# ma921/SOBER

Hardware: AMD Instinct MI355X
Metric: recombination-step candidates/sec (N_rec=100000, N_nys=500, d=10, batch=100) (higher is better)
Workload: dtype f64

## Files before the change

sober_amd/csrc/car.hip:

```cpp
#include "common.hpp"
#include <atomic>
#include <cstdlib>

namespace sober {

constexpr int CAR_MS = 7;
constexpr int CAR_CQ = 13;
constexpr int CAR_NS = 16 * CAR_CQ;
constexpr int CAR_PC = 128;
constexpr int CAR_BT = 256;

template <int CTRL>
__device__ __forceinline__ double dpp(double v) {
    int lo = __double2loint(v), hi = __double2hiint(v);
    lo = __builtin_amdgcn_mov_dpp(lo, CTRL, 0xf, 0xf, true);
    hi = __builtin_amdgcn_mov_dpp(hi, CTRL, 0xf, 0xf, true);
    return __hiloint2double(hi, lo);
}
constexpr int ROR1 = 0x121, ROR2 = 0x122, ROR4 = 0x124, ROR8 = 0x128;

#define CAR_LDS_BARRIER() do { __builtin_amdgcn_s_waitcnt(0xC07F); __builtin_amdgcn_s_barrier(); } while (0)

__device__ __forceinline__ double row16_sum(double v) {
    v += dpp<ROR8>(v);
    v += dpp<ROR4>(v);
    v += dpp<ROR2>(v);
    v += dpp<ROR1>(v);
    return v;
}
__device__ __forceinline__ double grp8_sum(double v) {
    v += dpp<ROR8>(v);
    v += dpp<ROR4>(v);
    v += dpp<ROR2>(v);
    return v;
}
__device__ __forceinline__ double rdlane(double v, int l) {
    const int lo = __builtin_amdgcn_readlane(__double2loint(v), l);
    const int hi = __builtin_amdgcn_readlane(__double2hiint(v), l);
    return __hiloint2double(hi, lo);
}
__device__ __forceinline__ double wave_sum(double v) {
    v = row16_sum(v);
    return ((rdlane(v, 0) + rdlane(v, 16)) + rdlane(v, 32)) + rdlane(v, 48);
}

template <int CTRL, int ROW_MASK>
__device__ __forceinline__ unsigned long long dpp_u64(unsigned long long v) {
    int lo = (int)(unsigned)v, hi = (int)(unsigned)(v >> 32);
    lo = __builtin_amdgcn_update_dpp(lo, lo, CTRL, ROW_MASK, 0xf, false);
    hi = __builtin_amdgcn_update_dpp(hi, hi, CTRL, ROW_MASK, 0xf, false);
    return ((unsigned long long)(unsigned)hi << 32) | (unsigned)lo;
}
constexpr int BCAST15 = 0x142, BCAST31 = 0x143;

__device__ __forceinline__ unsigned long long ratio_key(double x) {
    const unsigned long long b = (unsigned long long)__double_as_longlong(x);
    const unsigned long long k = (b >> 63) ? ~b : (b | 0x8000000000000000ull);
    return (x != x) ? 0ull : k;
}

__device__ __forceinline__ double car_rcp(double c) {
    double r = __builtin_amdgcn_rcp(c);
    double e = fma(-c, r, 1.0);
    r = fma(r, e, r);
    e = fma(-c, r, 1.0);
    return fma(r, e, r);
}
__device__ __forceinline__ void amin_take(double& best, int& piv, double ob, int op) {
    const bool bn = best != best, on = ob != ob;
    const bool lt = (ob < best) | ((ob == best) & (op < piv));
    const bool nn = on & ((!bn) | (op < piv));
    const bool take = (op >= 0) & ((piv < 0) | ((bn | on) ? nn : lt));
    best = take ? ob : best;
    piv = take ? op : piv;
}


typedef unsigned int car_u32x4 __attribute__((ext_vector_type(4)));
typedef unsigned int car_u32x2 __attribute__((ext_vector_type(2)));
typedef __amdgpu_buffer_rsrc_t car_rsrc_t;
constexpr unsigned CARF_ERR = 0, CARF_XCD = 16, CARF_TICKET = 32, CARF_PROGRESS = 48, CARF_DONE = 56;
__host__ __device__ constexpr int64_t carf_bytes(int) { return 64; }
constexpr unsigned CARF_SPIN_LIMIT = 1u << 22;
__device__ __forceinline__ void carf_put(car_rsrc_t rs, unsigned off, double v, unsigned tag) {
    car_u32x4 g;
    g.x = (unsigned)__double2loint(v); g.y = tag; g.z = (unsigned)__double2hiint(v); g.w = tag;
    __builtin_amdgcn_raw_buffer_store_b128(g, rs, off, 0, 0);
}
__device__ __forceinline__ car_u32x4 carf_load(car_rsrc_t rs, unsigned off) {
    return __builtin_amdgcn_raw_buffer_load_b128(rs, off, 0, 16);
}
__device__ __forceinline__ bool carf_ok(const car_u32x4& g, unsigned tag) { return (g.y == tag) & (g.w == tag); }
__device__ __forceinline__ double carf_val(const car_u32x4& g) { return __hiloint2double((int)g.z, (int)g.x); }
struct CarPub { car_rsrc_t rs; unsigned tag0; };
__device__ __forceinline__ void car_publish_progress(const CarPub& pub, int k) {
    const int tid = threadIdx.x;
    if (k > 0 && (tid >> 6) == (((k - 1) & 15) >> 2)) {
        __builtin_amdgcn_s_waitcnt(0x0F70);
        if ((tid & 63) == 0) __builtin_amdgcn_raw_buffer_store_b32(pub.tag0 + (unsigned)k, pub.rs, CARF_PROGRESS, 0, 0);
    }
}

#ifdef CAR_BSTAMPS
#define CB_DECL unsigned long long cacc_[10] = {0, 0, 0, 0, 0, 0, 0, 0, 0, 0}, ctl_; \
    asm volatile("s_memtime %0\n\ts_waitcnt lgkmcnt(0)" : "=s"(ctl_) :: "memory");
#define CB_STAMP(K) do { unsigned long long t_; asm volatile("s_memtime %0\n\ts_waitcnt lgkmcnt(0)" : "=s"(t_) :: "memory"); \
    cacc_[K] += t_ - ctl_; ctl_ = t_; } while (0)
#define CB_FLUSH(S_) do { if ((threadIdx.x & 63) == 0) for (int k_ = 0; k_ < 10; ++k_) \
    ((unsigned long long*)(taup + 128 + CAR_NS * CAR_PC))[((threadIdx.x >> 6) * 8 + (S_)) * 10 + k_] = cacc_[k_]; } while (0)
#else
#define CB_DECL
#define CB_STAMP(K) do { } while (0)
#define CB_FLUSH(S_) do { } while (0)
#endif

struct CarLds2 {
    double* rowg; double* colg; double* zpart; double* s2part; double* zsum; double* scal; double* hsc;
};

#define CB2_RSUM(v) row16_sum(v)
#define CB2_HUPD(n, o) (n)
#define CB2_GUPD(n, o) (n)
#define CB2_BARRIER() CAR_LDS_BARRIER()
#define CB2_VSTORE(e) e
#ifdef CAR_BSTAMPS
#define CB2_STAMP(K, VAL) do { unsigned long long t_; asm volatile("s_memtime %0\n\ts_waitcnt lgkmcnt(0)" : "=s"(t_), "+v"(VAL) :: "memory"); \
    cacc_[K] += t_ - ctl_; ctl_ = t_; } while (0)
#else
#define CB2_STAMP(K, VAL) do { } while (0)
#endif
template <int S, bool FUSED, int MS, int CQ>
__device__ __forceinline__ void car_bidiag2_block(double (&a)[CAR_MS][CAR_CQ], double (&colp)[CAR_MS], int m, const CarLds2& L,
                                                  double* __restrict__ vws, double* __restrict__ taup, const CarPub& pub) {
    const int tid = threadIdx.x;
    const int R = tid >> 4, C = tid & 15;
    const int i_end = min(16 * S + 16, m - 1);
    constexpr int S1 = (S + 1 < MS) ? S + 1 : S;
    const car_rsrc_t vrs = __builtin_amdgcn_make_buffer_rsrc(vws, 0, (int)((size_t)m * CAR_NS * sizeof(double)), 0x00020000);
    CB_DECL
    for (int i = 16 * S; i < i_end; ++i) {
        const int li = i & 15, p = i & 1, pp = p ^ 1;
        if constexpr (FUSED) car_publish_progress(pub, i);
        double z[CAR_CQ], x[CAR_CQ], f[CAR_MS], cur[CAR_MS];
        CB_STAMP(0);
        const double tauq = L.hsc[0], sc2 = L.hsc[1];
#pragma unroll
        for (int q = S; q < CQ; ++q) { x[q] = L.rowg[pp * CAR_NS + C + 16 * q]; z[q] = L.zsum[C + 16 * q]; }
        const double rgi = L.rowg[pp * CAR_NS + i];
#pragma unroll
        for (int k = S; k < MS; ++k) cur[k] = L.colg[pp * 128 + R + 16 * k];
#pragma unroll
        for (int q = S; q < CQ; ++q) {
            z[q] = fma(sc2, z[q], x[q]);
            x[q] = fma(-tauq, z[q], x[q]);
        }
        z[S] = (C >= li) ? z[S] : 0.0;
        x[S] = (C > li) ? x[S] : 0.0;
#pragma unroll
        for (int k = S; k < MS; ++k) f[k] = tauq * (sc2 * colp[k]);
        f[S] = (R == li) ? tauq : f[S];
        const double zi = rdlane(z[S], li);
        const double alpha = fma(-tauq, zi, rgi);
#pragma unroll
        for (int k = S; k < MS; ++k) cur[k] = fma(-f[k], zi, cur[k]);
#pragma unroll
        for (int q = S; q < CQ; ++q)
#pragma unroll
            for (int k = S; k < MS; ++k) a[k][q] = CB2_HUPD(fma(-f[k], z[q], a[k][q]), a[k][q]);
        double ss0 = 0.0, ss1 = 0.0;
#pragma unroll
        for (int q = S; q < CQ; ++q) { if (q & 1) ss1 = fma(x[q], x[q], ss1); else ss0 = fma(x[q], x[q], ss0); }
        double ss = CB2_RSUM(ss0 + ss1);
        CB2_STAMP(2, ss);
        double beta, tau, sc;
        larfg_vt(alpha, ss, tau, sc); (void)beta;
        CB2_STAMP(3, tau);
        double tG[CAR_MS];
#pragma unroll
        for (int k = S; k < MS; ++k) {
            double w0 = 0.0, w1 = 0.0;
#pragma unroll
            for (int q = S; q < CQ; ++q) { if (q & 1) w1 = fma(a[k][q], x[q], w1); else w0 = fma(a[k][q], x[q], w0); }
            tG[k] = tau * fma(sc, CB2_RSUM(w0 + w1), cur[k]);
        }
        tG[S] = (R > li) ? tG[S] : 0.0;
        CB2_STAMP(4, tG[S]);
#pragma unroll
        for (int k = S; k < MS; ++k) colp[k] = cur[k] - tG[k];
        colp[S] = (R > li) ? colp[S] : 0.0;
#pragma unroll
        for (int q = S; q < CQ; ++q) x[q] *= sc;
        if (R == li) {
            const unsigned so = (unsigned)__builtin_amdgcn_readfirstlane(i) * (unsigned)(CAR_NS * 8);
            unsigned c8 = (unsigned)C * 8u;
            asm volatile("" : "+v"(c8));
#pragma unroll
            for (int q = 0; q < CAR_CQ; ++q) {
                double v;
                if (q < S || q >= CQ) v = 0.0;
                else if (q == S) v = (C < li) ? 0.0 : ((C == li) ? 1.0 : x[S]);
                else v = x[q];
                car_u32x2 g;
                g.x = (unsigned)__double2loint(v); g.y = (unsigned)__double2hiint(v);
                CB2_VSTORE(__builtin_amdgcn_raw_buffer_store_b64(g, vrs, c8 + (unsigned)(128 * q), so, 0));
            }
            if (C == 0) taup[i] = tau;
        }
#pragma unroll
        for (int k = S; k < MS; ++k)
#pragma unroll
            for (int q = S; q < CQ; ++q) a[k][q] = CB2_GUPD(fma(-tG[k], x[q], a[k][q]), a[k][q]);
        const bool last = li == 15;
        const int n1 = (li + 1) & 15;
        if (!last) {
            if (R == n1) {
#pragma unroll
                for (int q = S; q < CQ; ++q) L.rowg[p * CAR_NS + C + 16 * q] = a[S][q];
                if (C == 0) L.scal[p] = colp[S];
            }
            if (C == n1) {
#pragma unroll
                for (int k = S; k < MS; ++k) L.colg[p * 128 + R + 16 * k] = a[k][S];
            }
        } else {
            if (R == 0) {
#pragma unroll
                for (int q = S; q < CQ; ++q) L.rowg[p * CAR_NS + C + 16 * q] = a[S1][q];
                if (C == 0) L.scal[p] = colp[S1];
            }
            if (C == 0) {
#pragma unroll
                for (int k = S; k < MS; ++k) L.colg[p * 128 + R + 16 * k] = a[k][S + 1];
            }
        }
        CB2_STAMP(5, a[S][S]);
        double cm[CAR_MS];
#pragma unroll
        for (int k = S; k < MS; ++k) cm[k] = colp[k];
        cm[S] = (R > li + 1) ? cm[S] : 0.0;
        if constexpr (S + 1 < MS) cm[S + 1] = (last && R == 0) ? 0.0 : cm[S + 1];
        double yp[CAR_CQ], s2p = 0.0;
#pragma unroll
        for (int q = S; q < CQ; ++q) yp[q] = cm[S] * a[S][q];
#pragma unroll
        for (int k = S + 1; k < MS; ++k)
#pragma unroll
            for (int q = S; q < CQ; ++q) yp[q] = fma(cm[k], a[k][q], yp[q]);
#pragma unroll
        for (int k = S; k < MS; ++k) s2p = fma(cm[k], cm[k], s2p);
#pragma unroll
        for (int q = S; q < CQ; ++q) L.zpart[R * CAR_NS + C + 16 * q] = yp[q];
        if (C == 0) L.s2part[R] = s2p;
        CB_STAMP(6);
        CB2_BARRIER();
        CB_STAMP(7);
        if (tid < 192) {
            const int c = 16 * S + tid;
            if (c < 16 * CQ) {
                double z0 = 0.0, z1 = 0.0;
#pragma unroll
                for (int w = 0; w < 16; w += 2) {
                    z0 += L.zpart[w * CAR_NS + c];
                    z1 += L.zpart[(w + 1) * CAR_NS + c];
                }
                L.zsum[c] = z0 + z1;
            }
        } else {
            if constexpr (S == 0) {
                if (tid < 16 * CQ) {
                    double z0 = 0.0, z1 = 0.0;
#pragma unroll
                    for (int w = 0; w < 16; w += 2) {
                        z0 += L.zpart[w * CAR_NS + tid];
                        z1 += L.zpart[(w + 1) * CAR_NS + tid];
                    }
                    L.zsum[tid] = z0 + z1;
                }
            }
            const double s2n = row16_sum(L.s2part[C]);
            double tq, s2c;
            larfg_vt(L.scal[p], s2n, tq, s2c);
            if (tid == 192) { L.hsc[0] = tq; L.hsc[1] = s2c; }
        }
        CB_STAMP(8);
        CB2_BARRIER();
        CB_STAMP(9);
    }
    CB_FLUSH(S);
}

template <int S, bool FUSED, int MS, int CQ>
__device__ __forceinline__ void car_bidiag2_last(int m, const CarLds2& L, double* __restrict__ vws, double* __restrict__ taup,
                                                 const CarPub& pub) {
    const int tid = threadIdx.x;
    const int R = tid >> 4, C = tid & 15;
    const int i = m - 1, li = i & 15, pp = (i & 1) ^ 1;
    if constexpr (FUSED) car_publish_progress(pub, i);
    double x[CAR_CQ], zS = 0.0;
    const double tauq = L.hsc[0], sc2 = L.hsc[1];
#pragma unroll
    for (int q = S; q < CQ; ++q) {
        const double rg = L.rowg[pp * CAR_NS + C + 16 * q];
        const double zq = fma(sc2, L.zsum[C + 16 * q], rg);
        if (q == S) zS = zq;
        x[q] = fma(-tauq, zq, rg);
    }
    x[S] = (C > li) ? x[S] : 0.0;
    const double zi = rdlane(zS, li);
    const double alpha = fma(-tauq, zi, L.rowg[pp * CAR_NS + i]);
    double ss0 = 0.0, ss1 = 0.0;
#pragma unroll
    for (int q = S; q < CQ; ++q) { if (q & 1) ss1 = fma(x[q], x[q], ss1); else ss0 = fma(x[q], x[q], ss0); }
    const double ss = row16_sum(ss0 + ss1);
    double beta, tau, sc;
    larfg_vt(alpha, ss, tau, sc); (void)beta;
    if (R == li) {
#pragma unroll
        for (int q = 0; q < CAR_CQ; ++q) {
            double v;
            if (q < S || q >= CQ) v = 0.0;
            else if (q == S) v = (C < li) ? 0.0 : ((C == li) ? 1.0 : x[S] * sc);
            else v = x[q] * sc;
            vws[(size_t)i * CAR_NS + C + 16 * q] = v;
        }
        if (C == 0) taup[i] = tau;
    }
}

template <bool FUSED, int MS, int CQ>
__device__ __forceinline__ void car_bidiag2_body(const double* __restrict__ X, int ldx, int N, int m,
                                                 double* __restrict__ vws, double* __restrict__ taup, const CarPub& pub) {
    __shared__ double rowg[2 * CAR_NS];
    __shared__ double colg[2 * 128];
    __shared__ double zpart[16 * CAR_NS];
    __shared__ double s2part[16];
    __shared__ double zsum[CAR_NS + 8];
    __shared__ double scal[2];
    __shared__ double hsc[2];
    const int tid = threadIdx.x;
    const int R = tid >> 4, C = tid & 15;
    double a[CAR_MS][CAR_CQ], colp[CAR_MS];
#pragma unroll
    for (int k = 0; k < CAR_MS; ++k) {
        colp[k] = 0.0;
#pragma unroll
        for (int q = 0; q < CAR_CQ; ++q) {
            const int r = R + 16 * k, c = C + 16 * q;
            a[k][q] = 0.0;
            if (k < MS && q < CQ) a[k][q] = (c < N && r < m) ? ((r == 0) ? 1.0 : X[(size_t)c * ldx + (r - 1)]) : 0.0;
        }
    }
    if (tid < CAR_NS) { rowg[CAR_NS + tid] = (tid < N) ? 1.0 : 0.0; zsum[tid] = 0.0; }
    if (tid < 128) colg[128 + tid] = (tid < m && N > 0) ? ((tid == 0) ? 1.0 : X[tid - 1]) : 0.0;
    if (tid < 8) zsum[CAR_NS + tid] = 0.0;
    if (tid < 2) { scal[tid] = 0.0; hsc[tid] = 0.0; }
    __syncthreads();
    const CarLds2 L{rowg, colg, zpart, s2part, zsum, scal, hsc};
    car_bidiag2_block<0, FUSED, MS, CQ>(a, colp, m, L, vws, taup, pub);
    if constexpr (MS > 1) if (m > 17) car_bidiag2_block<1, FUSED, MS, CQ>(a, colp, m, L, vws, taup, pub);
    if constexpr (MS > 2) if (m > 33) car_bidiag2_block<2, FUSED, MS, CQ>(a, colp, m, L, vws, taup, pub);
    if constexpr (MS > 3) if (m > 49) car_bidiag2_block<3, FUSED, MS, CQ>(a, colp, m, L, vws, taup, pub);
    if constexpr (MS > 4) if (m > 65) car_bidiag2_block<4, FUSED, MS, CQ>(a, colp, m, L, vws, taup, pub);
    if constexpr (MS > 5) if (m > 81) car_bidiag2_block<5, FUSED, MS, CQ>(a, colp, m, L, vws, taup, pub);
    if constexpr (MS > 6) if (m > 97) car_bidiag2_block<6, FUSED, MS, CQ>(a, colp, m, L, vws, taup, pub);
    const int sl = (m - 1) >> 4;
    if (sl == 0) car_bidiag2_last<0, FUSED, MS, CQ>(m, L, vws, taup, pub);
    if constexpr (MS > 1) if (sl == 1) car_bidiag2_last<1, FUSED, MS, CQ>(m, L, vws, taup, pub);
    if constexpr (MS > 2) if (sl == 2) car_bidiag2_last<2, FUSED, MS, CQ>(m, L, vws, taup, pub);
    if constexpr (MS > 3) if (sl == 3) car_bidiag2_last<3, FUSED, MS, CQ>(m, L, vws, taup, pub);
    if constexpr (MS > 4) if (sl == 4) car_bidiag2_last<4, FUSED, MS, CQ>(m, L, vws, taup, pub);
    if constexpr (MS > 5) if (sl == 5) car_bidiag2_last<5, FUSED, MS, CQ>(m, L, vws, taup, pub);
    if constexpr (MS > 6) if (sl >= 6) car_bidiag2_last<6, FUSED, MS, CQ>(m, L, vws, taup, pub);
}

template <int MS, int CQ>
__global__ __launch_bounds__(CAR_BT) void k_car_bidiag(const double* __restrict__ X, int ldx, int N, int m,
                                                       double* __restrict__ vws, double* __restrict__ taup) {
    car_bidiag2_body<false, MS, CQ>(X, ldx, N, m, vws, taup, CarPub{});
}

#ifdef SP_TSTAMPS
__device__ unsigned long long g_car_rt[8];
#define CAR_RT(K) do { unsigned long long t_; asm volatile("s_memrealtime %0\n\ts_waitcnt lgkmcnt(0)" : "=s"(t_) :: "memory"); g_car_rt[K] = t_; } while (0)
#define CAR_RT_MAX(K) do { unsigned long long t_; asm volatile("s_memrealtime %0\n\ts_waitcnt lgkmcnt(0)" : "=s"(t_) :: "memory"); atomicMax(&g_car_rt[K], t_); } while (0)
#else
#define CAR_RT(K) do { } while (0)
#define CAR_RT_MAX(K) do { } while (0)
#endif
template <int MS, int CQ>
__global__ __launch_bounds__(CAR_BT) void k_car_bidiag_fused(const double* __restrict__ X, int ldx, int N, int m,
                                                             double* __restrict__ vws, double* __restrict__ taup,
                                                             double* __restrict__ Phi, void* __restrict__ comm,
                                                             unsigned cbytes, unsigned epoch, unsigned spin_limit) {
    const car_rsrc_t rs = __builtin_amdgcn_make_buffer_rsrc(comm, 0, (int)cbytes, 0x00020000);
    const unsigned tag0 = epoch << 7;
    unsigned* words = (unsigned*)comm;
    const unsigned xcc = __builtin_amdgcn_s_getreg(20 | (0 << 6) | (3 << 11)) & 7u;
    if (blockIdx.x == 0) {
        if (threadIdx.x == 0) {
            __hip_atomic_store(words + CARF_ERR / 4, 0u, __ATOMIC_RELAXED, __HIP_MEMORY_SCOPE_AGENT);
            __hip_atomic_store(words + CARF_TICKET / 4, 0u, __ATOMIC_RELAXED, __HIP_MEMORY_SCOPE_AGENT);
            __hip_atomic_store(words + CARF_DONE / 4, 0u, __ATOMIC_RELAXED, __HIP_MEMORY_SCOPE_AGENT);
            __hip_atomic_store(words + CARF_XCD / 4, (epoch << 4) | (xcc + 1u), __ATOMIC_RELEASE, __HIP_MEMORY_SCOPE_AGENT);
        }
        const CarPub pub{rs, tag0};
#ifdef SP_TSTAMPS
        if (threadIdx.x == 0) { CAR_RT(0); g_car_rt[3] = 0ull; }
#endif
        car_bidiag2_body<true, MS, CQ>(X, ldx, N, m, vws, taup, pub);
        __syncthreads();
        if (threadIdx.x == 0) CAR_RT(1);
        car_publish_progress(pub, m);
        if (threadIdx.x == 0) CAR_RT(2);
        return;
    }
    __shared__ int s_group;
    const int tid = threadIdx.x, lane = tid & 63, wave = tid >> 6;
    if (tid == 0) {
        unsigned spins = 0, w;
        int grp = -1;
        while (((w = __hip_atomic_load(words + CARF_XCD / 4, __ATOMIC_ACQUIRE, __HIP_MEMORY_SCOPE_AGENT)) >> 4) != epoch) {
            if (++spins > CARF_SPIN_LIMIT) { w = 0; break; }
            __builtin_amdgcn_s_sleep(2);
        }
        if ((w & 15u) == xcc + 1u) grp = 0;
        s_group = grp;
    }
    __syncthreads();
    if (s_group < 0) return;
    const int NC = N - m;
    constexpr int RW = 2;
    constexpr int n_groups = CAR_NS / (4 * RW);
    static_assert(n_groups == CAR_NS / 8, "the pivot kernels check CARF_DONE against CAR_NS / 8");
    for (;;) {
        __syncthreads();
        if (tid == 0)
            s_group = (int)__hip_atomic_fetch_add(words + CARF_TICKET / 4, 1u, __ATOMIC_RELAXED, __HIP_MEMORY_SCOPE_AGENT);
        __syncthreads();
        const int grp = s_group;
        if (grp >= n_groups) return;
        const int r0 = (4 * grp + wave) * RW;
        double p[RW][4];
#pragma unroll
        for (int w = 0; w < RW; ++w)
#pragma unroll
            for (int q = 0; q < 4; ++q) p[w][q] = (lane + 64 * q == r0 + w) ? 1.0 : 0.0;
        const bool ok3 = lane + 192 < CAR_NS;
        bool failed = false;
        if (r0 < N) {
            const car_rsrc_t rv = __builtin_amdgcn_make_buffer_rsrc(vws, 0, (int)((size_t)(m * CAR_NS + 128) * sizeof(double)), 0x00020000);
            int have = 0;
            if (spin_limit == 0u) {
                __builtin_amdgcn_raw_buffer_store_b32(1, rs, CARF_ERR, 0, 16);
                failed = true;
            }
            for (int i = 0; i < m && !failed; ++i) {
                unsigned spins = 0;
                while (have <= i) {
                    const unsigned w = (unsigned)__builtin_amdgcn_raw_buffer_load_b32(rs, CARF_PROGRESS, 0, 16);
                    if ((w >> 7) == epoch) have = (int)(w & 127u);
                    if (have > i) break;
                    if (++spins > spin_limit ||
                        ((spins & 255u) == 0u && __builtin_amdgcn_raw_buffer_load_b32(rs, CARF_ERR, 0, 16) != 0)) {
                        __builtin_amdgcn_raw_buffer_store_b32(1, rs, CARF_ERR, 0, 16);
                        failed = true;
                        break;
                    }
                    __builtin_amdgcn_s_sleep(4);
                }
                if (failed) break;
                const unsigned base = (unsigned)(i * CAR_NS) * 8u;
                double vv[4];
#pragma unroll
                for (int q = 0; q < 4; ++q) {
                    const auto g2 = __builtin_amdgcn_raw_buffer_load_b64(rv, base + (unsigned)min(lane + 64 * q, CAR_NS - 1) * 8u, 0, 16);
                    vv[q] = __hiloint2double((int)g2[1], (int)g2[0]);
                }
                const auto gt2 = __builtin_amdgcn_raw_buffer_load_b64(rv, (unsigned)(m * CAR_NS + i) * 8u, 0, 16);
                const double tau = __hiloint2double((int)gt2[1], (int)gt2[0]);
                const double v0 = vv[0], v1 = vv[1], v2 = vv[2], v3 = ok3 ? vv[3] : 0.0;
                double d[RW];
#pragma unroll
                for (int w = 0; w < RW; ++w) d[w] = fma(v0, p[w][0], v1 * p[w][1]) + fma(v2, p[w][2], v3 * p[w][3]);
#pragma unroll
                for (int w = 0; w < RW; ++w) {
                    const double t = tau * wave_sum(d[w]);
                    p[w][0] = fma(-t, v0, p[w][0]); p[w][1] = fma(-t, v1, p[w][1]);
                    p[w][2] = fma(-t, v2, p[w][2]); p[w][3] = fma(-t, v3, p[w][3]);
                }
            }
        }
#pragma unroll
        for (int w = 0; w < RW; ++w) {
            const int r = r0 + w;
#pragma unroll
// ... 437 lines not shown
    const double al = w / wn;
    kmin[t] = ok ? ratio_key(al) : ~0ull;
    kidx[t] = t;
    __syncthreads();
    for (int h = 256; h > 0; h >>= 1) {
        if (t < h) {
            const unsigned long long a = kmin[t], b = kmin[t + h];
            if (b < a || (b == a && kidx[t + h] < kidx[t])) { kmin[t] = b; kidx[t] = kidx[t + h]; }
        }
        __syncthreads();
    }
    const bool any = kmin[0] != ~0ull;
    const int piv = kidx[0];
    __shared__ double s_al;
    if (t == piv) s_al = al;
    __syncthreads();
    double w2 = w;
    if (any && t < n1) w2 = (t == piv) ? 0.0 : __dsub_rn(w, __dmul_rn(s_al, wn));
    const bool keep = t < n1 && w2 > 0.0;
    cnt[t] = keep ? 1 : 0;
    __syncthreads();
    for (int h = 1; h < 512; h <<= 1) {
        const int v = (t >= h) ? cnt[t - h] : 0;
        __syncthreads();
        cnt[t] += v;
        __syncthreads();
    }
    if (keep) w_star[cnt[t] - 1] = w2;
    red[t] = keep ? (double)(cnt[t] - 1) : -1.0;
    __syncthreads();
    for (int sidx = t; sidx < Nsets; sidx += 512) {
        const int r1 = rank1[sidx];
        keep_rank[sidx] = (r1 >= 0 && r1 < n1) ? (int)red[r1] : -1;
    }
    if (t == 0) *n_keep_out = cnt[511];
}

}

extern "C" int sober_car_mc_supported(int N, int m);
extern "C" int64_t sober_car_mc_ws_bytes(int N, int m);
extern "C" int sober_car_mc_device(const double* X, int ldx, int N, int m, const double* mu_in, int32_t* keep_rank,
                                   double* w_star, int32_t* n_keep, double* mu_out, double* phi_out, void* ws,
                                   int64_t ws_bytes, void* stream);
extern "C" int sober_car_big_supported(int N, int m);
extern "C" int64_t sober_car_big_ws_bytes(int N, int m);
extern "C" int sober_car_big_device(const double* X, int ldx, int N, int m, const double* mu_in, int32_t* keep_rank,
                                    double* w_star, int32_t* n_keep, double* mu_out, double* phi_out, void* ws,
                                    int64_t ws_bytes, void* stream);

static int car_one_cu(int N, int m) {
    return (m >= 2 && N > m && N <= sober::CAR_NS && m <= 16 * sober::CAR_MS && N - m <= sober::SP_W * sober::SP_BC) ? 1 : 0;
}

extern "C" int sober_car_supported(int N, int m) {
    return (car_one_cu(N, m) || sober_car_mc_supported(N, m) || sober_car_big_supported(N, m)) ? 1 : 0;
}

extern "C" int64_t sober_car_ws_bytes(int N, int m) {
    const int64_t one = ((int64_t)m * sober::CAR_NS + 128 + (int64_t)sober::CAR_NS * sober::CAR_PC + 512) * (int64_t)sizeof(double)
                        + sober::carf_bytes(0);
    if (car_one_cu(N, m)) return one;
    int64_t need = sober_car_big_supported(N, m) ? sober_car_big_ws_bytes(N, m) : 0;
    if (need < one) need = one;
    if (sober_car_mc_supported(N < m + 1 ? N : m + 1, m)) { const int64_t mc = sober_car_mc_ws_bytes(N, m); if (mc > need) need = mc; }
    return need;
}

static int car_pivot_attr(size_t sp_bytes) {
    static std::atomic<unsigned long long> done{0};
    if (sober_attr_needed(done)) {
        HIP_TRY(hipFuncSetAttribute((const void*)sober::k_car_pivot_stream<1>, hipFuncAttributeMaxDynamicSharedMemorySize, (int)sp_bytes));
        HIP_TRY(hipFuncSetAttribute((const void*)sober::k_car_pivot_stream<2>, hipFuncAttributeMaxDynamicSharedMemorySize, (int)sp_bytes));
        HIP_TRY(hipFuncSetAttribute((const void*)sober::k_car_pivot_stream<4>, hipFuncAttributeMaxDynamicSharedMemorySize, (int)sp_bytes));
        sober_attr_done(done);
    }
    return 0;
}

extern "C" int sober_car_giveup_forced(void) { return sober::switches().car_force_giveup ? 1 : 0; }

extern "C" int sober_car_safe_supported(int N, int m) { return (car_one_cu(N, m) || sober_car_big_supported(N, m)) ? 1 : 0; }

#define CAR_BY_SIZE(m_, N_, LAUNCH)                                                                    \
    do {                                                                                               \
        if ((m_) <= 16 && (N_) <= 32) { constexpr int MS_ = 1, CQ_ = 2; LAUNCH; }                      \
        else if ((m_) <= 32 && (N_) <= 64) { constexpr int MS_ = 2, CQ_ = 4; LAUNCH; }                 \
        else if ((m_) <= 64 && (N_) <= 112) { constexpr int MS_ = 4, CQ_ = 7; LAUNCH; }                \
        else if ((N_) <= 112) { constexpr int MS_ = sober::CAR_MS, CQ_ = 7; LAUNCH; }                  \
        else { constexpr int MS_ = sober::CAR_MS, CQ_ = sober::CAR_CQ; LAUNCH; }                       \
    } while (0)

#define CAR_PIVOT_BY_SIZE(N_, LAUNCH)                                  \
    do {                                                               \
        if ((N_) <= 64) { constexpr int NQ_ = 1; LAUNCH; }             \
        else if ((N_) <= 128) { constexpr int NQ_ = 2; LAUNCH; }       \
        else { constexpr int NQ_ = 4; LAUNCH; }                        \
    } while (0)

namespace sober {
__global__ __launch_bounds__(256) void k_probe_rcp(const double* __restrict__ x, double* __restrict__ out, int64_t n) {
    const int64_t i = (int64_t)blockIdx.x * 256 + threadIdx.x;
    if (i < n) out[i] = __builtin_amdgcn_rcp(x[i]);
}
}
extern "C" int sober_probe_rcp(const double* x, double* out, int64_t n, void* stream) {
    if (n < 0 || (n > 0 && (!x || !out))) return SOBER_E_ARG;
    if (n == 0) return 0;
    hipLaunchKernelGGL(sober::k_probe_rcp, dim3((unsigned)((n + 255) / 256)), dim3(256), 0, (hipStream_t)stream, x, out, n);
    LAUNCH_CHECK();
    return 0;
}

extern "C" int sober_car_device_ex(const double* X, int ldx, int N, int m, const double* mu_in,
                                   int32_t* keep_rank, double* w_star, int32_t* n_keep, double* mu_out,
                                   double* phi_out, void* ws, int64_t ws_bytes, int mode, void* stream) {
    if (!X || !mu_in || !keep_rank || !w_star || !n_keep || !mu_out || !ws || ldx < m - 1) return SOBER_E_ARG;
    if (mode != SOBER_CAR_DEFAULT && mode != SOBER_CAR_SAFE) return SOBER_E_ARG;
    if (!car_one_cu(N, m)) {
        if (mode == SOBER_CAR_DEFAULT && sober_car_mc_supported(N, m))
            return sober_car_mc_device(X, ldx, N, m, mu_in, keep_rank, w_star, n_keep, mu_out, phi_out, ws, ws_bytes, stream);
        return sober_car_big_device(X, ldx, N, m, mu_in, keep_rank, w_star, n_keep, mu_out, phi_out, ws, ws_bytes, stream);
    }
    if (ws_bytes < sober_car_ws_bytes(N, m)) return SOBER_E_WS;
    hipStream_t st = (hipStream_t)stream;
    double* vws = (double*)ws;
    double* taup = vws + (size_t)m * sober::CAR_NS;
    double* Phi = taup + 128;
    const bool unfused = sober::switches().car_unfused;
    const size_t sp_bytes = sizeof(sober::SpSlot) * sober::SP_RING + sober::SP_W * sizeof(int);
    { const int rc = car_pivot_attr(sp_bytes); if (rc != 0) return rc; }
    if (phi_out != nullptr || unfused || mode == SOBER_CAR_SAFE) {
        CAR_BY_SIZE(m, N, hipLaunchKernelGGL((sober::k_car_bidiag<MS_, CQ_>), dim3(1), dim3(sober::CAR_BT), 0, st, X, ldx, N, m, vws, taup));
        LAUNCH_CHECK();
        hipLaunchKernelGGL(sober::k_car_phi, dim3(sober::CAR_PC / 4), dim3(256), 0, st, vws, taup, N, m, Phi, phi_out);
        LAUNCH_CHECK();
        CAR_PIVOT_BY_SIZE(N, hipLaunchKernelGGL((sober::k_car_pivot_stream<NQ_>), dim3(1), dim3(sober::SP_W * 64), sp_bytes, st, Phi, N, m,
                                                mu_in, keep_rank, w_star, n_keep, mu_out, (const unsigned*)nullptr, (int)sober::switches().car_exact_ratio));
        LAUNCH_CHECK();
        return 0;
    }
    static std::atomic<unsigned> epoch_ctr{0};
    const unsigned epoch = (epoch_ctr.fetch_add(1) + 1u) & 0x1FFFFFFu;
    void* comm = (void*)(Phi + (size_t)sober::CAR_NS * sober::CAR_PC + 512);
    constexpr int per_xcd = 40;
    const unsigned spin_limit = sober_car_giveup_forced() ? 0u : sober::CARF_SPIN_LIMIT;
    CAR_BY_SIZE(m, N, hipLaunchKernelGGL((sober::k_car_bidiag_fused<MS_, CQ_>), dim3(1 + 8 * per_xcd), dim3(sober::CAR_BT), 0, st, X, ldx,
                                         N, m, vws, taup, Phi, comm, (unsigned)sober::carf_bytes(0), epoch, spin_limit));
    LAUNCH_CHECK();
    CAR_PIVOT_BY_SIZE(N, hipLaunchKernelGGL((sober::k_car_pivot_stream<NQ_>), dim3(1), dim3(sober::SP_W * 64), sp_bytes, st, Phi, N, m,
                                            mu_in, keep_rank, w_star, n_keep, mu_out, (const unsigned*)comm, (int)sober::switches().car_exact_ratio));
    LAUNCH_CHECK();
    return 0;
}

extern "C" int sober_car_device(const double* X, int ldx, int N, int m, const double* mu_in,
                                int32_t* keep_rank, double* w_star, int32_t* n_keep, double* mu_out,
                                double* phi_out, void* ws, int64_t ws_bytes, void* stream) {
    return sober_car_device_ex(X, ldx, N, m, mu_in, keep_rank, w_star, n_keep, mu_out, phi_out, ws, ws_bytes,
                               SOBER_CAR_DEFAULT, stream);
}

extern "C" int sober_second_elimination(const double* phi, const double* objp, const double* w1, const int32_t* rank1,
                                        int n1, int Nsets, int32_t* keep_rank, double* w_star, int32_t* n_keep,
                                        void* stream) {
    if (!phi || !objp || !w1 || !rank1 || !keep_rank || !w_star || !n_keep || n1 <= 0 || Nsets <= 0) return SOBER_E_ARG;
    if (n1 > 512) return SOBER_E_DIM;
    hipLaunchKernelGGL(sober::k_second_elim<false>, dim3(1), dim3(512), 0, (hipStream_t)stream, phi, objp, w1, rank1, n1, Nsets,
                       keep_rank, w_star, n_keep, (const int32_t*)nullptr, (const int32_t*)nullptr);
    LAUNCH_CHECK();
    return 0;
}

extern "C" int sober_second_elimination_rows(const double* null_row, const double* obj_row, const double* w1,
                                             const int32_t* rank1, const int32_t* n_keep1, const int32_t* status, int n1,
                                             int Nsets, int32_t* keep_rank, double* w_star, int32_t* n_keep, void* stream) {
    if (!null_row || !obj_row || !w1 || !rank1 || !n_keep1 || !keep_rank || !w_star || !n_keep || n1 <= 0 || Nsets <= 0)
        return SOBER_E_ARG;
    if (n1 > 512) return SOBER_E_DIM;
    hipLaunchKernelGGL(sober::k_second_elim<true>, dim3(1), dim3(512), 0, (hipStream_t)stream, null_row, obj_row, w1, rank1, n1,
                       Nsets, keep_rank, w_star, n_keep, n_keep1, status);
    LAUNCH_CHECK();
    return 0;
}

#ifdef SP_TSTAMPS
extern "C" int sober_debug_sp_stamps(unsigned long long* out260) {
    return (int)hipMemcpyFromSymbol(out260, HIP_SYMBOL(sober::g_sp_stamps), sizeof(unsigned long long) * 260, 0, hipMemcpyDeviceToHost);
}
extern "C" int sober_debug_car_rt(unsigned long long* out8) {
    return (int)hipMemcpyFromSymbol(out8, HIP_SYMBOL(sober::g_car_rt), sizeof(unsigned long long) * 8, 0, hipMemcpyDeviceToHost);
}
extern "C" int sober_debug_sp_segments(unsigned long long* out128) {
    return (int)hipMemcpyFromSymbol(out128, HIP_SYMBOL(sober::g_sp_seg), sizeof(unsigned long long) * 128, 0, hipMemcpyDeviceToHost);
}
#endif
```

sober_amd/csrc/misc.hip:

```cpp
#include "common.hpp"
#include "internal.hpp"

namespace sober {

__global__ void k_scale_points(const double* __restrict__ X, int64_t n, int d, int64_t ldx,
                               const double* __restrict__ ls, int ls_len, double* __restrict__ out,
                               int dt) {
    const int64_t t = (int64_t)blockIdx.x * blockDim.x + threadIdx.x;
    if (t >= n * dt) return;
    const int64_t i = t / dt;
    const int j = (int)(t % dt);
    double v = 0.0;
    if (j < d) v = X[i * ldx + j] / ls[ls_len == 1 ? 0 : j];
    out[t] = v;
}

__global__ void k_scale_points2(const double* __restrict__ Xa, int64_t na, int64_t lda, const double* __restrict__ Xb, int64_t nb,
                                int64_t ldb, int d, const double* __restrict__ ls, int ls_len, double* __restrict__ out, int dt) {
    const int64_t t = (int64_t)blockIdx.x * blockDim.x + threadIdx.x;
    if (t >= (na + nb) * dt) return;
    const int64_t i = t / dt;
    const int j = (int)(t % dt);
    double v = 0.0;
    if (j < d) v = (i < na ? Xa[i * lda + j] : Xb[(i - na) * ldb + j]) / ls[ls_len == 1 ? 0 : j];
// ... 393 lines not shown
constexpr int CW_BLOCKS = 256, CW_THREADS = 256;

__global__ __launch_bounds__(CW_THREADS) void k_clean_partial(double* __restrict__ w, int64_t n,
                                                              double eps, double* __restrict__ part) {
    __shared__ double s[CW_THREADS];
    double acc = 0.0;
    for (int64_t i = (int64_t)blockIdx.x * CW_THREADS + threadIdx.x; i < n;
         i += (int64_t)CW_BLOCKS * CW_THREADS) {
        double v = w[i];
        if (v < eps) v = 0.0;
        if (isinf(v)) v = eps;
        if (isnan(v)) v = eps;
        w[i] = v;
        acc += v;
    }
    s[threadIdx.x] = acc;
    __syncthreads();
    for (int o = CW_THREADS / 2; o > 0; o >>= 1) {
        if (threadIdx.x < o) s[threadIdx.x] += s[threadIdx.x + o];
        __syncthreads();
    }
    if (threadIdx.x == 0) part[blockIdx.x] = s[0];
}

__global__ __launch_bounds__(CW_BLOCKS) void k_clean_scale(double* __restrict__ w, int64_t n, const double* __restrict__ part) {
    __shared__ double s[CW_BLOCKS];
    s[threadIdx.x] = part[threadIdx.x];
    __syncthreads();
    for (int o = CW_BLOCKS / 2; o > 0; o >>= 1) {
        if (threadIdx.x < o) s[threadIdx.x] += s[threadIdx.x + o];
        __syncthreads();
    }
    const double tot = s[0];
    const int64_t i = (int64_t)blockIdx.x * blockDim.x + threadIdx.x;
    if (i >= n) return;
    w[i] = (tot != 0.0) ? w[i] / tot : 1.0 / (double)n;
}

__global__ void k_wkde_draw(const double* __restrict__ eps, int64_t n, int d, const int32_t* __restrict__ comp,
                            const double* __restrict__ Xobs, int ldx, const double* __restrict__ L,
                            const double* __restrict__ lo, const double* __restrict__ hi,
                            double* __restrict__ x, int32_t* __restrict__ inside) {
    extern __shared__ double sL[];
    for (int t = threadIdx.x; t < d * d; t += blockDim.x) sL[t] = L[t];
    __syncthreads();
    const int64_t r = (int64_t)blockIdx.x * blockDim.x + threadIdx.x;
    if (r >= n) return;
    const double* e = eps + r * d;
    const double* loc = Xobs + (size_t)comp[r] * ldx;
    bool ok = true;
    for (int k = 0; k < d; ++k) {
        double acc = 0.0;
        for (int j = 0; j <= k; ++j) acc = fma(sL[k * d + j], e[j], acc);
        const double v = loc[k] + acc;
        x[r * d + k] = v;
        if (lo) ok = ok && !(v < lo[k]) && !(v > hi[k]);
    }
    if (inside) inside[r] = ok ? 1 : 0;
}

}

#include <cstdlib>
using namespace sober;

static inline unsigned nblk(int64_t n, int b) { return (unsigned)((n + b - 1) / b); }

extern "C" int sober_abi_version(void) { return SOBER_ABI_VERSION; }
extern "C" int sober_diag_build(void) {
#ifdef SOBER_DIAG_BUILD
    return 1;
#else
    return 0;
#endif
}

namespace sober {
static Switches read_switches() {
    Switches w;
    w.level_two_launches = getenv("SOBER_LEVEL_TWO_LAUNCHES") != nullptr;
    w.tani_no_queue = getenv("SOBER_TANI_NO_QUEUE") != nullptr;
    w.car_force_giveup = getenv("SOBER_CAR_FORCE_GIVEUP") != nullptr;
    w.car_unfused = getenv("SOBER_CAR_UNFUSED") != nullptr;
    w.level_no_classes = getenv("SOBER_LEVEL_NO_CLASSES") != nullptr;
    w.car_exact_ratio = getenv("SOBER_CAR_EXACT_RATIO") != nullptr;
    return w;
}
static Switches g_switches = read_switches();
const Switches& switches() { return g_switches; }
}
extern "C" int sober_reload_switches(void) { sober::g_switches = sober::read_switches(); return 0; }
namespace sober {
LaunchEvents& launch_events() {
    static thread_local LaunchEvents le;
    return le;
}
}
extern "C" int sober_set_launch_events(void* start, void* stop) {
    if ((start == nullptr) != (stop == nullptr)) return SOBER_E_ARG;
    sober::launch_events() = sober::LaunchEvents{(hipEvent_t)start, (hipEvent_t)stop};
    return 0;
}

extern "C" int sober_padded_dim(int d) {
    if (d <= 0) return SOBER_E_ARG;
    const int dts[] = {4, 8, 12, 16, 20, 24, 32};
    for (int v : dts)
        if (d <= v) return v;
    return SOBER_E_DIM;
}

extern "C" int sober_bit_words(int d) {
    if (d <= 0) return SOBER_E_ARG;
    const int w = (d + 63) / 64;
    const int ws[] = {1, 2, 4, 8, 16, 32};
    for (int v : ws)
        if (w <= v) return v;
    return SOBER_E_DIM;
}

__global__ void k_box_muller(const double* __restrict__ u, int64_t numel, double* __restrict__ out) {
    const int64_t t = (int64_t)blockIdx.x * blockDim.x + threadIdx.x;
    const int64_t full = numel / 16;
    const bool tail = (numel % 16) != 0;
    const int64_t npairs = (full + (tail ? 1 : 0)) * 8;
    if (t >= npairs) return;
    const int64_t g = t >> 3;
    const int j = (int)(t & 7);
    const bool is_tail = g == full;
    const int64_t ub = is_tail ? numel : g * 16, ob = is_tail ? numel - 16 : g * 16;
    const double u1 = 1.0 - u[ub + j], u2 = u[ub + j + 8];
    const double radius = sqrt(-2.0 * log(u1));
    const double theta = 6.283185307179586 * u2;
    double sn, cs;
    sincos(theta, &sn, &cs);
    const int64_t keep_below = tail ? numel - 16 : numel;
    if (is_tail || ob + j < keep_below) out[ob + j] = radius * cs;
    if (is_tail || ob + j + 8 < keep_below) out[ob + j + 8] = radius * sn;
}

extern "C" int sober_box_muller(const double* u, int64_t numel, double* out, void* stream) {
    if (!u || !out || numel < 16) return SOBER_E_ARG;
    const int64_t npairs = ((numel + 15) / 16) * 8;
    hipLaunchKernelGGL(k_box_muller, dim3(nblk(npairs, 256)), dim3(256), 0, (hipStream_t)stream, u, numel, out);
    LAUNCH_CHECK();
    return 0;
}

extern "C" int sober_scale_points(const double* X, int64_t n, int d, int64_t ldx,
                                  const double* lengthscale, int ls_len, double* out, int dt,
                                  void* stream) {
    if (!X || !lengthscale || !out || n <= 0 || d <= 0 || dt < d || ldx < d) return SOBER_E_ARG;
    if (ls_len != 1 && ls_len != d) return SOBER_E_ARG;
    hipLaunchKernelGGL(k_scale_points, dim3(nblk(n * dt, 256)), dim3(256), 0, (hipStream_t)stream, X,
                       n, d, ldx, lengthscale, ls_len, out, dt);
    LAUNCH_CHECK();
    return 0;
}

int sober::scale_points2(const double* Xa, int64_t na, int64_t lda, const double* Xb, int64_t nb, int64_t ldb, int d,
                         const double* lengthscale, int ls_len, double* out, int dt, void* stream) {
    if (!Xa || !Xb || !lengthscale || !out || na <= 0 || nb <= 0 || d <= 0 || dt < d || lda < d || ldb < d) return SOBER_E_ARG;
    if (ls_len != 1 && ls_len != d) return SOBER_E_ARG;
    hipLaunchKernelGGL(k_scale_points2, dim3(nblk((na + nb) * dt, 256)), dim3(256), 0, (hipStream_t)stream, Xa, na, lda, Xb, nb,
                       ldb, d, lengthscale, ls_len, out, dt);
    LAUNCH_CHECK();
// ... 332 lines not shown
```

sober_amd/csrc/switches.hpp:

```cpp
#pragma once
namespace sober {
struct Switches {
    bool level_two_launches;
    bool tani_no_queue;
    bool car_force_giveup;
    bool car_unfused;
    bool car_exact_ratio;
    bool level_no_classes;
};
const Switches& switches();
}
```

Before: 26.97 million.

## Shift CAR bidiagonalization start by eight rows/cols within register tile

Adds a compile-time shift SH=8 that offsets the matrix inside the 16-row/column register tile so the Householder sweep starts mid-block, with index remapping for the V workspace, taup, progress publishing and the zpart reduction order. It also fuses the colp update into the tG loop as an fma. The shift is enabled by default when the sizes fit, and an env switch turns it off. The aim is likely to change which block stages run or how they align for the batch sizes used. It adds index arithmetic and doubles the template instantiations, and the wraparound store offsets and the XOR-ordered reduction could introduce correctness or rounding differences.

Result: slower. 26.54 million (-1.6%).

```diff
diff --git a/sober_amd/csrc/car.hip b/sober_amd/csrc/car.hip
--- a/sober_amd/csrc/car.hip
+++ b/sober_amd/csrc/car.hip
@@ -93,11 +93,12 @@
 __device__ __forceinline__ bool carf_ok(const car_u32x4& g, unsigned tag) { return (g.y == tag) & (g.w == tag); }
 __device__ __forceinline__ double carf_val(const car_u32x4& g) { return __hiloint2double((int)g.z, (int)g.x); }
 struct CarPub { car_rsrc_t rs; unsigned tag0; };
+template <int SH>
 __device__ __forceinline__ void car_publish_progress(const CarPub& pub, int k) {
     const int tid = threadIdx.x;
-    if (k > 0 && (tid >> 6) == (((k - 1) & 15) >> 2)) {
+    if (k > SH && (tid >> 6) == (((k - 1) & 15) >> 2)) {
         __builtin_amdgcn_s_waitcnt(0x0F70);
-        if ((tid & 63) == 0) __builtin_amdgcn_raw_buffer_store_b32(pub.tag0 + (unsigned)k, pub.rs, CARF_PROGRESS, 0, 0);
+        if ((tid & 63) == 0) __builtin_amdgcn_raw_buffer_store_b32(pub.tag0 + (unsigned)(k - SH), pub.rs, CARF_PROGRESS, 0, 0);
     }
 }
 
@@ -129,18 +130,18 @@
 #else
 #define CB2_STAMP(K, VAL) do { } while (0)
 #endif
-template <int S, bool FUSED, int MS, int CQ>
+template <int S, bool FUSED, int MS, int CQ, int SH>
 __device__ __forceinline__ void car_bidiag2_block(double (&a)[CAR_MS][CAR_CQ], double (&colp)[CAR_MS], int m, const CarLds2& L,
                                                   double* __restrict__ vws, double* __restrict__ taup, const CarPub& pub) {
     const int tid = threadIdx.x;
     const int R = tid >> 4, C = tid & 15;
     const int i_end = min(16 * S + 16, m - 1);
     constexpr int S1 = (S + 1 < MS) ? S + 1 : S;
-    const car_rsrc_t vrs = __builtin_amdgcn_make_buffer_rsrc(vws, 0, (int)((size_t)m * CAR_NS * sizeof(double)), 0x00020000);
+    const car_rsrc_t vrs = __builtin_amdgcn_make_buffer_rsrc(vws, 0, (int)((size_t)(m - SH) * CAR_NS * sizeof(double)), 0x00020000);
     CB_DECL
-    for (int i = 16 * S; i < i_end; ++i) {
+    for (int i = (S == 0) ? SH : 16 * S; i < i_end; ++i) {
         const int li = i & 15, p = i & 1, pp = p ^ 1;
-        if constexpr (FUSED) car_publish_progress(pub, i);
+        if constexpr (FUSED) car_publish_progress<SH>(pub, i);
         double z[CAR_CQ], x[CAR_CQ], f[CAR_MS], cur[CAR_MS];
         CB_STAMP(0);
         const double tauq = L.hsc[0], sc2 = L.hsc[1];
@@ -181,19 +182,21 @@
             double w0 = 0.0, w1 = 0.0;
 #pragma unroll
             for (int q = S; q < CQ; ++q) { if (q & 1) w1 = fma(a[k][q], x[q], w1); else w0 = fma(a[k][q], x[q], w0); }
-            tG[k] = tau * fma(sc, CB2_RSUM(w0 + w1), cur[k]);
+            const double wv = fma(sc, CB2_RSUM(w0 + w1), cur[k]);
+            tG[k] = tau * wv;
+            colp[k] = fma(-tau, wv, cur[k]);
         }
         tG[S] = (R > li) ? tG[S] : 0.0;
         CB2_STAMP(4, tG[S]);
-#pragma unroll
-        for (int k = S; k < MS; ++k) colp[k] = cur[k] - tG[k];
         colp[S] = (R > li) ? colp[S] : 0.0;
 #pragma unroll
         for (int q = S; q < CQ; ++q) x[q] *= sc;
         if (R == li) {
-            const unsigned so = (unsigned)__builtin_amdgcn_readfirstlane(i) * (unsigned)(CAR_NS * 8);
+            const unsigned so = (unsigned)__builtin_amdgcn_readfirstlane(i - SH) * (unsigned)(CAR_NS * 8);
             unsigned c8 = (unsigned)C * 8u;
             asm volatile("" : "+v"(c8));
+            unsigned c8w = c8;
+            if constexpr (SH > 0) c8w = (C < SH) ? c8 + (unsigned)(8 * (CAR_NS - SH)) : c8 - (unsigned)(8 * SH);
 #pragma unroll
             for (int q = 0; q < CAR_CQ; ++q) {
                 double v;
@@ -202,9 +205,10 @@
                 else v = x[q];
                 car_u32x2 g;
                 g.x = (unsigned)__double2loint(v); g.y = (unsigned)__double2hiint(v);
-                CB2_VSTORE(__builtin_amdgcn_raw_buffer_store_b64(g, vrs, c8 + (unsigned)(128 * q), so, 0));
+                const unsigned off = (q == 0) ? c8w : c8 + (unsigned)(128 * q - 8 * SH);
+                CB2_VSTORE(__builtin_amdgcn_raw_buffer_store_b64(g, vrs, off, so, 0));
             }
-            if (C == 0) taup[i] = tau;
+            if (C == 0) taup[i - SH] = tau;
         }
 #pragma unroll
         for (int k = S; k < MS; ++k)
@@ -260,8 +264,8 @@
                 double z0 = 0.0, z1 = 0.0;
 #pragma unroll
                 for (int w = 0; w < 16; w += 2) {
-                    z0 += L.zpart[w * CAR_NS + c];
-                    z1 += L.zpart[(w + 1) * CAR_NS + c];
+                    z0 += L.zpart[(w ^ SH) * CAR_NS + c];
+                    z1 += L.zpart[((w + 1) ^ SH) * CAR_NS + c];
                 }
                 L.zsum[c] = z0 + z1;
             }
@@ -271,8 +275,8 @@
                     double z0 = 0.0, z1 = 0.0;
 #pragma unroll
                     for (int w = 0; w < 16; w += 2) {
-                        z0 += L.zpart[w * CAR_NS + tid];
-                        z1 += L.zpart[(w + 1) * CAR_NS + tid];
+                        z0 += L.zpart[(w ^ SH) * CAR_NS + tid];
+                        z1 += L.zpart[((w + 1) ^ SH) * CAR_NS + tid];
                     }
                     L.zsum[tid] = z0 + z1;
                 }
@@ -289,13 +293,13 @@
     CB_FLUSH(S);
 }
 
-template <int S, bool FUSED, int MS, int CQ>
+template <int S, bool FUSED, int MS, int CQ, int SH>
 __device__ __forceinline__ void car_bidiag2_last(int m, const CarLds2& L, double* __restrict__ vws, double* __restrict__ taup,
                                                  const CarPub& pub) {
     const int tid = threadIdx.x;
     const int R = tid >> 4, C = tid & 15;
     const int i = m - 1, li = i & 15, pp = (i & 1) ^ 1;
-    if constexpr (FUSED) car_publish_progress(pub, i);
+    if constexpr (FUSED) car_publish_progress<SH>(pub, i);
     double x[CAR_CQ], zS = 0.0;
     const double tauq = L.hsc[0], sc2 = L.hsc[1];
 #pragma unroll
@@ -321,13 +325,14 @@
             if (q < S || q >= CQ) v = 0.0;
             else if (q == S) v = (C < li) ? 0.0 : ((C == li) ? 1.0 : x[S] * sc);
             else v = x[q] * sc;
-            vws[(size_t)i * CAR_NS + C + 16 * q] = v;
-        }
-        if (C == 0) taup[i] = tau;
-    }
-}
-
-template <bool FUSED, int MS, int CQ>
+            const int c = C + 16 * q - SH;
+            vws[(size_t)(i - SH) * CAR_NS + ((c < 0) ? c + CAR_NS : c)] = v;
+        }
+        if (C == 0) taup[i - SH] = tau;
+    }
+}
+
+template <bool FUSED, int MS, int CQ, int SH>
 __device__ __forceinline__ void car_bidiag2_body(const double* __restrict__ X, int ldx, int N, int m,
                                                  double* __restrict__ vws, double* __restrict__ taup, const CarPub& pub) {
     __shared__ double rowg[2 * CAR_NS];
@@ -345,38 +350,39 @@
         colp[k] = 0.0;
 #pragma unroll
         for (int q = 0; q < CAR_CQ; ++q) {
-            const int r = R + 16 * k, c = C + 16 * q;
+            const int r = R + 16 * k - SH, c = C + 16 * q - SH;
             a[k][q] = 0.0;
-            if (k < MS && q < CQ) a[k][q] = (c < N && r < m) ? ((r == 0) ? 1.0 : X[(size_t)c * ldx + (r - 1)]) : 0.0;
-        }
-    }
-    if (tid < CAR_NS) { rowg[CAR_NS + tid] = (tid < N) ? 1.0 : 0.0; zsum[tid] = 0.0; }
-    if (tid < 128) colg[128 + tid] = (tid < m && N > 0) ? ((tid == 0) ? 1.0 : X[tid - 1]) : 0.0;
+            if (k < MS && q < CQ) a[k][q] = (c >= 0 && c < N && r >= 0 && r < m) ? ((r == 0) ? 1.0 : X[(size_t)c * ldx + (r - 1)]) : 0.0;
+        }
+    }
+    if (tid < CAR_NS) { rowg[CAR_NS + tid] = (tid >= SH && tid - SH < N) ? 1.0 : 0.0; zsum[tid] = 0.0; }
+    if (tid < 128) colg[128 + tid] = (tid >= SH && tid - SH < m && N > 0) ? ((tid == SH) ? 1.0 : X[tid - SH - 1]) : 0.0;
     if (tid < 8) zsum[CAR_NS + tid] = 0.0;
     if (tid < 2) { scal[tid] = 0.0; hsc[tid] = 0.0; }
     __syncthreads();
     const CarLds2 L{rowg, colg, zpart, s2part, zsum, scal, hsc};
-    car_bidiag2_block<0, FUSED, MS, CQ>(a, colp, m, L, vws, taup, pub);
-    if constexpr (MS > 1) if (m > 17) car_bidiag2_block<1, FUSED, MS, CQ>(a, colp, m, L, vws, taup, pub);
-    if constexpr (MS > 2) if (m > 33) car_bidiag2_block<2, FUSED, MS, CQ>(a, colp, m, L, vws, taup, pub);
-    if constexpr (MS > 3) if (m > 49) car_bidiag2_block<3, FUSED, MS, CQ>(a, colp, m, L, vws, taup, pub);
-    if constexpr (MS > 4) if (m > 65) car_bidiag2_block<4, FUSED, MS, CQ>(a, colp, m, L, vws, taup, pub);
-    if constexpr (MS > 5) if (m > 81) car_bidiag2_block<5, FUSED, MS, CQ>(a, colp, m, L, vws, taup, pub);
-    if constexpr (MS > 6) if (m > 97) car_bidiag2_block<6, FUSED, MS, CQ>(a, colp, m, L, vws, taup, pub);
-    const int sl = (m - 1) >> 4;
-    if (sl == 0) car_bidiag2_last<0, FUSED, MS, CQ>(m, L, vws, taup, pub);
-    if constexpr (MS > 1) if (sl == 1) car_bidiag2_last<1, FUSED, MS, CQ>(m, L, vws, taup, pub);
-    if constexpr (MS > 2) if (sl == 2) car_bidiag2_last<2, FUSED, MS, CQ>(m, L, vws, taup, pub);
-    if constexpr (MS > 3) if (sl == 3) car_bidiag2_last<3, FUSED, MS, CQ>(m, L, vws, taup, pub);
-    if constexpr (MS > 4) if (sl == 4) car_bidiag2_last<4, FUSED, MS, CQ>(m, L, vws, taup, pub);
-    if constexpr (MS > 5) if (sl == 5) car_bidiag2_last<5, FUSED, MS, CQ>(m, L, vws, taup, pub);
-    if constexpr (MS > 6) if (sl >= 6) car_bidiag2_last<6, FUSED, MS, CQ>(m, L, vws, taup, pub);
-}
-
-template <int MS, int CQ>
+    const int mt = m + SH;
+    car_bidiag2_block<0, FUSED, MS, CQ, SH>(a, colp, mt, L, vws, taup, pub);
+    if constexpr (MS > 1) if (mt > 17) car_bidiag2_block<1, FUSED, MS, CQ, SH>(a, colp, mt, L, vws, taup, pub);
+    if constexpr (MS > 2) if (mt > 33) car_bidiag2_block<2, FUSED, MS, CQ, SH>(a, colp, mt, L, vws, taup, pub);
+    if constexpr (MS > 3) if (mt > 49) car_bidiag2_block<3, FUSED, MS, CQ, SH>(a, colp, mt, L, vws, taup, pub);
+    if constexpr (MS > 4) if (mt > 65) car_bidiag2_block<4, FUSED, MS, CQ, SH>(a, colp, mt, L, vws, taup, pub);
+    if constexpr (MS > 5) if (mt > 81) car_bidiag2_block<5, FUSED, MS, CQ, SH>(a, colp, mt, L, vws, taup, pub);
+    if constexpr (MS > 6) if (mt > 97) car_bidiag2_block<6, FUSED, MS, CQ, SH>(a, colp, mt, L, vws, taup, pub);
+    const int sl = (mt - 1) >> 4;
+    if (sl == 0) car_bidiag2_last<0, FUSED, MS, CQ, SH>(mt, L, vws, taup, pub);
+    if constexpr (MS > 1) if (sl == 1) car_bidiag2_last<1, FUSED, MS, CQ, SH>(mt, L, vws, taup, pub);
+    if constexpr (MS > 2) if (sl == 2) car_bidiag2_last<2, FUSED, MS, CQ, SH>(mt, L, vws, taup, pub);
+    if constexpr (MS > 3) if (sl == 3) car_bidiag2_last<3, FUSED, MS, CQ, SH>(mt, L, vws, taup, pub);
+    if constexpr (MS > 4) if (sl == 4) car_bidiag2_last<4, FUSED, MS, CQ, SH>(mt, L, vws, taup, pub);
+    if constexpr (MS > 5) if (sl == 5) car_bidiag2_last<5, FUSED, MS, CQ, SH>(mt, L, vws, taup, pub);
+    if constexpr (MS > 6) if (sl >= 6) car_bidiag2_last<6, FUSED, MS, CQ, SH>(mt, L, vws, taup, pub);
+}
+
+template <int MS, int CQ, int SH>
 __global__ __launch_bounds__(CAR_BT) void k_car_bidiag(const double* __restrict__ X, int ldx, int N, int m,
                                                        double* __restrict__ vws, double* __restrict__ taup) {
-    car_bidiag2_body<false, MS, CQ>(X, ldx, N, m, vws, taup, CarPub{});
+    car_bidiag2_body<false, MS, CQ, SH>(X, ldx, N, m, vws, taup, CarPub{});
 }
 
 #ifdef SP_TSTAMPS
@@ -387,7 +393,7 @@
 #define CAR_RT(K) do { } while (0)
 #define CAR_RT_MAX(K) do { } while (0)
 #endif
-template <int MS, int CQ>
+template <int MS, int CQ, int SH>
 __global__ __launch_bounds__(CAR_BT) void k_car_bidiag_fused(const double* __restrict__ X, int ldx, int N, int m,
                                                              double* __restrict__ vws, double* __restrict__ taup,
                                                              double* __restrict__ Phi, void* __restrict__ comm,
@@ -407,10 +413,10 @@
 #ifdef SP_TSTAMPS
         if (threadIdx.x == 0) { CAR_RT(0); g_car_rt[3] = 0ull; }
 #endif
-        car_bidiag2_body<true, MS, CQ>(X, ldx, N, m, vws, taup, pub);
+        car_bidiag2_body<true, MS, CQ, SH>(X, ldx, N, m, vws, taup, pub);
         __syncthreads();
         if (threadIdx.x == 0) CAR_RT(1);
-        car_publish_progress(pub, m);
+        car_publish_progress<SH>(pub, m + SH);
         if (threadIdx.x == 0) CAR_RT(2);
         return;
     }
@@ -1014,13 +1020,25 @@
 
 extern "C" int sober_car_safe_supported(int N, int m) { return (car_one_cu(N, m) || sober_car_big_supported(N, m)) ? 1 : 0; }
 
+#define CAR_SHIFT_OK(m_, N_) (!sober::switches().car_unshifted && (m_) + 8 <= 16 * MS_ && (N_) + 8 <= 16 * CQ_)
 #define CAR_BY_SIZE(m_, N_, LAUNCH)                                                                    \
     do {                                                                                               \
-        if ((m_) <= 16 && (N_) <= 32) { constexpr int MS_ = 1, CQ_ = 2; LAUNCH; }                      \
-        else if ((m_) <= 32 && (N_) <= 64) { constexpr int MS_ = 2, CQ_ = 4; LAUNCH; }                 \
-        else if ((m_) <= 64 && (N_) <= 112) { constexpr int MS_ = 4, CQ_ = 7; LAUNCH; }                \
-        else if ((N_) <= 112) { constexpr int MS_ = sober::CAR_MS, CQ_ = 7; LAUNCH; }                  \
-        else { constexpr int MS_ = sober::CAR_MS, CQ_ = sober::CAR_CQ; LAUNCH; }                       \
+        if ((m_) <= 16 && (N_) <= 32) {                                                                \
+            constexpr int MS_ = 1, CQ_ = 2;                                                            \
+            if (CAR_SHIFT_OK(m_, N_)) { constexpr int SH_ = 8; LAUNCH; } else { constexpr int SH_ = 0; LAUNCH; } \
+        } else if ((m_) <= 32 && (N_) <= 64) {                                                         \
+            constexpr int MS_ = 2, CQ_ = 4;                                                            \
+            if (CAR_SHIFT_OK(m_, N_)) { constexpr int SH_ = 8; LAUNCH; } else { constexpr int SH_ = 0; LAUNCH; } \
+        } else if ((m_) <= 64 && (N_) <= 112) {                                                        \
+            constexpr int MS_ = 4, CQ_ = 7;                                                            \
+            if (CAR_SHIFT_OK(m_, N_)) { constexpr int SH_ = 8; LAUNCH; } else { constexpr int SH_ = 0; LAUNCH; } \
+        } else if ((N_) <= 112) {                                                                      \
+            constexpr int MS_ = sober::CAR_MS, CQ_ = 7;                                                \
+            if (CAR_SHIFT_OK(m_, N_)) { constexpr int SH_ = 8; LAUNCH; } else { constexpr int SH_ = 0; LAUNCH; } \
+        } else {                                                                                       \
+            constexpr int MS_ = sober::CAR_MS, CQ_ = sober::CAR_CQ;                                    \
+            if (CAR_SHIFT_OK(m_, N_)) { constexpr int SH_ = 8; LAUNCH; } else { constexpr int SH_ = 0; LAUNCH; } \
+        }                                                                                              \
     } while (0)
 
 #define CAR_PIVOT_BY_SIZE(N_, LAUNCH)                                  \
@@ -1063,7 +1081,7 @@
     const size_t sp_bytes = sizeof(sober::SpSlot) * sober::SP_RING + sober::SP_W * sizeof(int);
     { const int rc = car_pivot_attr(sp_bytes); if (rc != 0) return rc; }
     if (phi_out != nullptr || unfused || mode == SOBER_CAR_SAFE) {
-        CAR_BY_SIZE(m, N, hipLaunchKernelGGL((sober::k_car_bidiag<MS_, CQ_>), dim3(1), dim3(sober::CAR_BT), 0, st, X, ldx, N, m, vws, taup));
+        CAR_BY_SIZE(m, N, hipLaunchKernelGGL((sober::k_car_bidiag<MS_, CQ_, SH_>), dim3(1), dim3(sober::CAR_BT), 0, st, X, ldx, N, m, vws, taup));
         LAUNCH_CHECK();
         hipLaunchKernelGGL(sober::k_car_phi, dim3(sober::CAR_PC / 4), dim3(256), 0, st, vws, taup, N, m, Phi, phi_out);
         LAUNCH_CHECK();
@@ -1077,7 +1095,7 @@
     void* comm = (void*)(Phi + (size_t)sober::CAR_NS * sober::CAR_PC + 512);
     constexpr int per_xcd = 40;
     const unsigned spin_limit = sober_car_giveup_forced() ? 0u : sober::CARF_SPIN_LIMIT;
-    CAR_BY_SIZE(m, N, hipLaunchKernelGGL((sober::k_car_bidiag_fused<MS_, CQ_>), dim3(1 + 8 * per_xcd), dim3(sober::CAR_BT), 0, st, X, ldx,
+    CAR_BY_SIZE(m, N, hipLaunchKernelGGL((sober::k_car_bidiag_fused<MS_, CQ_, SH_>), dim3(1 + 8 * per_xcd), dim3(sober::CAR_BT), 0, st, X, ldx,
                                          N, m, vws, taup, Phi, comm, (unsigned)sober::carf_bytes(0), epoch, spin_limit));
     LAUNCH_CHECK();
     CAR_PIVOT_BY_SIZE(N, hipLaunchKernelGGL((sober::k_car_pivot_stream<NQ_>), dim3(1), dim3(sober::SP_W * 64), sp_bytes, st, Phi, N, m,
diff --git a/sober_amd/csrc/misc.hip b/sober_amd/csrc/misc.hip
--- a/sober_amd/csrc/misc.hip
+++ b/sober_amd/csrc/misc.hip
@@ -499,6 +499,7 @@
     w.tani_no_queue = getenv("SOBER_TANI_NO_QUEUE") != nullptr;
     w.car_force_giveup = getenv("SOBER_CAR_FORCE_GIVEUP") != nullptr;
     w.car_unfused = getenv("SOBER_CAR_UNFUSED") != nullptr;
+    w.car_unshifted = getenv("SOBER_CAR_UNSHIFTED") != nullptr;
     w.level_no_classes = getenv("SOBER_LEVEL_NO_CLASSES") != nullptr;
     w.car_exact_ratio = getenv("SOBER_CAR_EXACT_RATIO") != nullptr;
     return w;
diff --git a/sober_amd/csrc/switches.hpp b/sober_amd/csrc/switches.hpp
--- a/sober_amd/csrc/switches.hpp
+++ b/sober_amd/csrc/switches.hpp
@@ -5,6 +5,7 @@
     bool tani_no_queue;
     bool car_force_giveup;
     bool car_unfused;
+    bool car_unshifted;
     bool car_exact_ratio;
     bool level_no_classes;
 };
```
